# kuldeepbrd1/graspLDM

Measured on AMD Instinct MI355X. Metric: grasps/sec whole-node (1024-pt cloud, 100 DDIM steps), higher is better.
Workload: dtype f32 (GEMMs as split-f16 x3 partial products on the f16 matrix pipe, f32 accumulation; GroupNorm / LayerNorm / attention / scheduler in f32); 1 GPU; LDM mode, 256 synthetic 1024-pt clouds per GPU x 20 grasps, 100 DDIM steps: BASELINE.json configs[2] per GPU (configs[3] = this per-GPU workload on 8 GPUs); experiment=fpc, clouds_per_gpu=256, grasps_per_cloud=20, points=1024, ddim_steps=100, encoder=PVCNNEncoder (shipped fpc config), parallelism=cloud-sharded x1, weights=synthetic recipe seed 0, streams=3

## Files before the change

### graspldm_amd/csrc/conv3d.hip

```cpp
#include "mfma_core.h"
#include "voxel_geom.h"

namespace {

#ifdef GLDM_DEBUG_KNOBS
__device__ long long g_c3_stamp[32];
#define GLDM_C3_STAMP(i) \
  do { if (blockIdx.x == 5 && blockIdx.y == (gridDim.y >> 1) && threadIdx.x == 0) g_c3_stamp[i] = (long long)__builtin_readcyclecounter(); } while (0)
#else
#define GLDM_C3_STAMP(i) do {} while (0)
#endif

template <int CTRL>
__device__ __forceinline__ float c3_dpp_mov(float x) {
  return __int_as_float(__builtin_amdgcn_update_dpp(0, __float_as_int(x), CTRL, 0xf, 0xf, false));
}
__device__ __forceinline__ float row16_sum(float x) {
  x += c3_dpp_mov<0xB1>(x);
  x += c3_dpp_mov<0x4E>(x);
  x += c3_dpp_mov<0x141>(x);
  x += c3_dpp_mov<0x140>(x);
  return x;
}

constexpr int kConvThreads = 256;

__host__ __device__ constexpr bool brick_vec4(int r) { return r <= 24; }
__host__ __device__ constexpr int brick_zp(int r) { return brick_vec4(r) ? r + 8 : r + 2; }
__host__ __device__ constexpr int brick_row_stride(int r) {
  return ((6 * 6 * brick_zp(r) + 31) / 32 * 32 + 16) - 32 >= 6 * 6 * brick_zp(r) ? (6 * 6 * brick_zp(r) + 31) / 32 * 32 - 16
                                                                                 : (6 * 6 * brick_zp(r) + 31) / 32 * 32 + 16;
}

template <int MT, int NTW, int JN>
__global__ __launch_bounds__(kConvThreads, 2) void conv3d_k3_kernel(const float *__restrict__ x,
                                                                    const float *__restrict__ wp,
                                                                    const float *__restrict__ bias, int cin, int cout,
                                                                    int r_arg, float *__restrict__ y,
                                                                    float *__restrict__ partial, int cout_total, int co0,
                                                                    int out_cl) {
  constexpr int r = 4 * NTW;
  (void)r_arg;
  extern __shared__ float lds[];
  __builtin_amdgcn_s_setprio(3);
  GLDM_C3_STAMP(0);
  const int tid = threadIdx.x, wave = tid >> 6, lane = tid & 63;
  const int col = lane & 15, kq = lane >> 4;
  const int bpr = r / kBrick;
  const int bx0 = (blockIdx.x / bpr) * kBrick, by0 = (blockIdx.x % bpr) * kBrick;
  const int b = blockIdx.y;
  constexpr bool kVec = brick_vec4(r);
  constexpr int r3 = r * r * r, zp = brick_zp(r), bv = 36 * zp, bvp = brick_row_stride(r);
  const int cblocks = (cin + 15) >> 4, kblocks = 27 * cblocks;
  x += (size_t)b * cin * r3;
  y += out_cl ? (size_t)b * cout_total * r3 + co0 : ((size_t)b * cout_total + co0) * r3;
  const WStream wv(wp, lane);
  const lds_f *l3 = (const lds_f *)lds;

  int obase[NTW], gvox[NTW];
#pragma unroll
  for (int ni = 0; ni < NTW; ++ni) {
    const int o = 16 * (wave * NTW + ni) + col;
    const int iz = o % r, ixy = o / r, ix = ixy >> 2, iy = ixy & 3;
    obase[ni] = (ix * 6 + iy) * zp + iz + (kVec ? 3 : 0) + kq * bvp;
    gvox[ni] = ((bx0 + ix) * r + by0 + iy) * r + iz;
  }
  f32x4 acc[MT][NTW];
#pragma unroll
  for (int mi = 0; mi < MT; ++mi) {
    f32x4 bvv;
#pragma unroll
    for (int q = 0; q < 4; ++q) bvv[q] = bias[min(16 * mi + 4 * kq + q, cout - 1)];
#pragma unroll
    for (int ni = 0; ni < NTW; ++ni) acc[mi][ni] = bvv;
  }

  constexpr int kSlotsRow = r / 4, kSlots = 36 * kSlotsRow;
  static_assert(!kVec || kSlots <= kConvThreads, "one interior slot per thread");
  constexpr int SQ = kVec ? 1 : (36 * (4 * NTW + 2) + kConvThreads - 1) / kConvThreads;
  constexpr int kStageCh = JN == 1 ? 4 : 16;
  int s_lds[SQ], s_glb[SQ];
#pragma unroll
  for (int q = 0; q < SQ; ++q) {
    const int rem = tid + q * kConvThreads;
    s_lds[q] = -1;
    s_glb[q] = -1;
    if (kVec) {
      if (rem < kSlots) {
        const int ixy = rem / kSlotsRow, k = rem - ixy * kSlotsRow;
        const int gx = bx0 + ixy / 6 - 1, gy = by0 + ixy % 6 - 1;
        s_lds[q] = ixy * zp + 4 * (k + 1);
        if ((unsigned)gx < (unsigned)r && (unsigned)gy < (unsigned)r) s_glb[q] = (gx * r + gy) * r + 4 * k;
      }
    } else if (rem < bv) {
      s_lds[q] = rem;
      const int ixy = rem / zp, izp = rem - ixy * zp;
      const int gx = bx0 + ixy / 6 - 1, gy = by0 + ixy % 6 - 1, gz = izp - 1;
      if ((unsigned)gx < (unsigned)r && (unsigned)gy < (unsigned)r && (unsigned)gz < (unsigned)r)
        s_glb[q] = (gx * r + gy) * r + gz;
    }
  }
  if constexpr (kVec) {
    const f32x4 z4 = f32x4{0.f, 0.f, 0.f, 0.f};
    if (tid < 72) {
      float *lc = lds + (tid >> 1) * zp + ((tid & 1) ? 4 * (kSlotsRow + 1) : 0);
#pragma unroll
      for (int ci = 0; ci < kStageCh; ++ci) *reinterpret_cast<f32x4 *>(lc + ci * bvp) = z4;
    }
    if (s_lds[0] >= 0 && s_glb[0] < 0) {
      float *lc = lds + s_lds[0];
#pragma unroll
      for (int ci = 0; ci < kStageCh; ++ci) *reinterpret_cast<f32x4 *>(lc + ci * bvp) = z4;
    }
  }
  float stg[kVec ? 1 : SQ][kVec ? 1 : kStageCh];
  f32x4 stv[kVec ? kStageCh : 1];
  const __amdgpu_buffer_rsrc_t xrs = __builtin_amdgcn_make_buffer_rsrc(const_cast<float *>(x), 0, cin * r3 * 4, 0x00020000);
  auto stage_load = [&](int cb) {
    if constexpr (kVec) {
      const int g0 = s_glb[0] >= 0 ? s_glb[0] : 0;
#pragma unroll
      for (int ci = 0; ci < kStageCh; ++ci)
        stv[ci] = __builtin_bit_cast(f32x4, __builtin_amdgcn_raw_buffer_load_b128(xrs, ((cb * 16 + ci) * r3 + g0) * 4, 0, 0));
    } else {
      const float *xc = x + (size_t)(cb * 16) * r3;
#pragma unroll
      for (int q = 0; q < SQ; ++q)
#pragma unroll
        for (int ci = 0; ci < kStageCh; ++ci) {
          stg[q][ci] = 0.f;
          if (s_glb[q] >= 0 && cb * 16 + ci < cin) stg[q][ci] = xc[(size_t)ci * r3 + s_glb[q]];
        }
    }
  };
  auto stage_store = [&]() {
    if constexpr (kVec) {
      if (s_glb[0] >= 0) {
        float *lc = lds + s_lds[0];
#pragma unroll
        for (int ci = 0; ci < kStageCh; ++ci) *reinterpret_cast<f32x4 *>(lc + ci * bvp) = stv[ci];
      }
    } else {
#pragma unroll
      for (int q = 0; q < SQ; ++q)
        if (s_lds[q] >= 0) {
          float *lc = lds + s_lds[q];
#pragma unroll
          for (int ci = 0; ci < kStageCh; ++ci) lc[ci * bvp] = stg[q][ci];
        }
    }
  };
  constexpr int kStageLoads = SQ * kStageCh;
  constexpr bool kLate = r <= 12 && kStageLoads <= 32;
  constexpr bool kPipe = SQ <= 4;
  GLDM_C3_STAMP(1);
  if (kPipe) stage_load(0);
  GLDM_C3_STAMP(2);
  for (int cb = 0; cb < cblocks; ++cb) {
    __syncthreads();
    if (cb < 3) GLDM_C3_STAMP(3 + 4 * cb);
    if (!kPipe) stage_load(cb);
    stage_store();
    if (cb < 3) GLDM_C3_STAMP(4 + 4 * cb);
    if (kPipe && !kLate && cb + 1 < cblocks) stage_load(cb + 1);
    __builtin_amdgcn_sched_barrier(0);
    __syncthreads();
    if (cb < 3) GLDM_C3_STAMP(5 + 4 * cb);
    f32x4 a_cur[MT], a_nxt[MT];
#pragma unroll
    for (int mi = 0; mi < MT; ++mi) a_cur[mi] = wv[((size_t)mi * kblocks + cb) * 64];
    float bf[NTW], bn[NTW];
#pragma unroll
    for (int ni = 0; ni < NTW; ++ni) bf[ni] = l3[obase[ni]];
    __builtin_amdgcn_s_setprio(0);
    for (int tap = 0; tap < 27; ++tap) {
#ifdef GLDM_DEBUG_KNOBS
      if (cb < 2 && (tap == 1 || tap == 2 || tap == 14)) GLDM_C3_STAMP(14 + 3 * cb + (tap == 1 ? 0 : (tap == 2 ? 1 : 2)));
#endif
      if (kLate && tap == 25 && cb + 1 < cblocks) stage_load(cb + 1);
      const int tn = tap + 1 < 27 ? tap + 1 : tap;
#pragma unroll
      for (int mi = 0; mi < MT; ++mi) a_nxt[mi] = wv[((size_t)mi * kblocks + tn * cblocks + cb) * 64];
      __builtin_amdgcn_sched_barrier(0);
      const int toff = ((tap / 9) * 6 + (tap / 3) % 3) * zp + tap % 3;
      const int tnoff = ((tn / 9) * 6 + (tn / 3) % 3) * zp + tn % 3;
#pragma unroll
      for (int j = 0; j < JN; ++j) {
        const int noff = j + 1 < JN ? toff + 4 * (j + 1) * bvp : tnoff;
#pragma unroll
        for (int ni = 0; ni < NTW; ++ni) bn[ni] = l3[obase[ni] + noff];
#pragma unroll
        for (int mi = 0; mi < MT; ++mi)
#pragma unroll
          for (int ni = 0; ni < NTW; ++ni)
            acc[mi][ni] = __builtin_amdgcn_mfma_f32_16x16x4f32(a_cur[mi][j], bf[ni], acc[mi][ni], 0, 0, 0);
#pragma unroll
        for (int ni = 0; ni < NTW; ++ni) bf[ni] = bn[ni];
      }
#pragma unroll
      for (int mi = 0; mi < MT; ++mi) a_cur[mi] = a_nxt[mi];
    }
    __builtin_amdgcn_s_setprio(3);
    if (cb < 3) GLDM_C3_STAMP(6 + 4 * cb);
  }
  __syncthreads();
  GLDM_C3_STAMP(20);
  float *s_part = lds;
#pragma unroll
  for (int mi = 0; mi < MT; ++mi) {
#pragma unroll
    for (int q = 0; q < 4; ++q) {
      const int co = 16 * mi + 4 * kq + q;
      float s = 0.f, s2 = 0.f;
#pragma unroll
      for (int ni = 0; ni < NTW; ++ni) {
        const float v = acc[mi][ni][q];
        s += v;
        s2 += v * v;
      }
      s = row16_sum(s);
      s2 = row16_sum(s2);
      if (col == 0 && co < cout) {
        s_part[(wave * MT * 16 + co) * 2] = s;
        s_part[(wave * MT * 16 + co) * 2 + 1] = s2;
      }
    }
  }
  GLDM_C3_STAMP(24);
  __syncthreads();
  GLDM_C3_STAMP(25);
  if (tid < cout) {
    float s = 0.f, s2 = 0.f;
    for (int w = 0; w < 4; ++w) {
      s += s_part[(w * MT * 16 + tid) * 2];
      s2 += s_part[(w * MT * 16 + tid) * 2 + 1];
    }
    float *p = partial + (((size_t)b * gridDim.x + blockIdx.x) * cout_total + co0 + tid) * 2;
    p[0] = s;
    p[1] = s2;
  }
  GLDM_C3_STAMP(26);
  if (out_cl) {
#pragma unroll
    for (int ni = 0; ni < NTW; ++ni)
#pragma unroll
      for (int mi = 0; mi < MT; ++mi)
        if (16 * mi + 4 * kq < cout) *reinterpret_cast<f32x4 *>(y + (size_t)gvox[ni] * cout_total + 16 * mi + 4 * kq) = acc[mi][ni];
  } else {
#pragma unroll
    for (int mi = 0; mi < MT; ++mi)
#pragma unroll
      for (int q = 0; q < 4; ++q) {
        const int co = 16 * mi + 4 * kq + q;
        if (co < cout) {
#pragma unroll
          for (int ni = 0; ni < NTW; ++ni) y[(size_t)co * r3 + gvox[ni]] = acc[mi][ni][q];
        }
      }
  }
  GLDM_C3_STAMP(21);
}


constexpr int kPairs = 14;

__device__ __forceinline__ float c3_wave_max(float x) {
#pragma unroll
  for (int off = 32; off >= 1; off >>= 1) x = fmaxf(x, __shfl_xor(x, off, 64));
  return x;
}

template <int MT, int R, int ZB, int WAVES, bool ACT = false>
__global__ __launch_bounds__(64 * WAVES, (ZB * 16 / WAVES / 16 >= 6) ? 1 : 2) void conv3d_k3_pl_kernel(const float *__restrict__ x,
                                                                                      const float *__restrict__ wp3,
                                                                                      const float *__restrict__ bias, int cin,
                                                                                      int cout, float *__restrict__ y,
                                                                                      float *__restrict__ partial,
                                                                                      const float *__restrict__ in_coef,
                                                                                      int out_cl) {
  constexpr int r = R, NTW = ZB / WAVES, kThreads = 64 * WAVES, kZParts = R / ZB;
  constexpr int GM = MT % 3 == 0 ? 3 : (MT % 4 == 0 ? 4 : (MT % 2 == 0 ? 2 : 1));
  constexpr int GN = NTW % 3 == 0 ? 3 : (NTW % 2 == 0 ? 2 : 1);
  static_assert(R % ZB == 0 && ZB % WAVES == 0, "whole n-tiles per wave");
  constexpr int MG = MT / GM, NG = NTW / GN;
  constexpr int zp = ZB + 2, nvox = 36 * zp, r3 = r * r * r;
  constexpr int hs = (nvox + 15) & ~15;
  constexpr int kItems = 2 * nvox, kRounds = (kItems + kThreads - 1) / kThreads;
  constexpr bool kDB = R == 24 && ZB == 24;
  constexpr bool kRanged = !ACT;
  extern __shared__ float lds[];
  GLDM_C3_STAMP(0);
  __builtin_amdgcn_s_setprio(3);
  const int tid = threadIdx.x, wave = tid >> 6, lane = tid & 63;
  const int col = lane & 15, kq = lane >> 4;
  const int bpr = r / kBrick;
  const int bxy = blockIdx.x / kZParts, bz0 = (blockIdx.x % kZParts) * ZB;
  const int bx0 = (bxy / bpr) * kBrick, by0 = (bxy % bpr) * kBrick;
  const int b = blockIdx.y;
  const int cblocks = (cin + 15) >> 4, kblocks = kPairs * cblocks;
  x += (size_t)b * cin * r3;
  y += (size_t)b * cout * r3;
  const WStream wv(wp3, lane);
  constexpr int kSet = kSplit * 2 * hs;
  lds_u4 *pl0 = (lds_u4 *)lds;

  int vb[NTW];
#pragma unroll
  for (int ni = 0; ni < NTW; ++ni) {
    const int o = 16 * (wave * NTW + ni) + col;
    const int iz = o % ZB, ixy = o / ZB, ix = ixy >> 2, iy = ixy & 3;
    vb[ni] = (ix * 6 + iy) * zp + iz + (kq & 1) * hs;
  }
  f32x4 acc[MT][NTW];
#pragma unroll
  for (int mi = 0; mi < MT; ++mi) {
    f32x4 bvv;
#pragma unroll
    for (int q = 0; q < 4; ++q) bvv[q] = bias[16 * mi + 4 * kq + q];
#pragma unroll
    for (int ni = 0; ni < NTW; ++ni) acc[mi][ni] = bvv;
  }
  int s_lds[kRounds], s_glb[kRounds];
#pragma unroll
  for (int q = 0; q < kRounds; ++q) {
    const int it = tid + q * kThreads;
    s_lds[q] = -1;
    s_glb[q] = -1;
    if (it < kItems) {
      const int h = it / nvox, v = it - h * nvox;
      const int ixy = v / zp, izp = v - ixy * zp;
      const int gx = bx0 + ixy / 6 - 1, gy = by0 + ixy % 6 - 1, gz = bz0 + izp - 1;
      s_lds[q] = h * hs + v;
      if ((unsigned)gx < (unsigned)r && (unsigned)gy < (unsigned)r && (unsigned)gz < (unsigned)r)
        s_glb[q] = (gx * r + gy) * r + gz + 8 * h * r3;
    }
  }
  {
    const u32x4 z4 = u32x4{0u, 0u, 0u, 0u};
#pragma unroll
    for (int q = 0; q < kRounds; ++q)
      if (s_lds[q] >= 0 && s_glb[q] < 0) {
#pragma unroll
        for (int k = 0; k < kSplit; ++k) {
          pl0[k * 2 * hs + s_lds[q]] = z4;
          if constexpr (kDB) pl0[kSet + k * 2 * hs + s_lds[q]] = z4;
        }
      }
  }
  float stg[kRounds][8];
  auto stage_load = [&](int cb) {
    const float *xc = x + (size_t)(cb * 16) * r3;
#pragma unroll
    for (int q = 0; q < kRounds; ++q) {
      const int g0 = s_glb[q] >= 0 ? s_glb[q] : 0;
#pragma unroll
      for (int j = 0; j < 8; ++j) stg[q][j] = xc[(size_t)j * r3 + g0];
    }
  };
  float *s_coef = lds + (kDB ? 2 : 1) * kSet * 4;
  if constexpr (ACT) {
    for (int i = tid; i < 2 * cin; i += kThreads) s_coef[i] = in_coef[(size_t)b * cin * 2 + i];
  }
  unsigned s_run_u = 0x3f800000u;
  float *rng = s_coef;
  auto stage_store = [&](int cb) {
    lds_u4 *pl = pl0 + (kDB ? (cb & 1) * kSet : 0);
#pragma unroll
    for (int q = 0; q < kRounds; ++q)
      if (s_glb[q] >= 0) {
        if constexpr (kRanged) {
          const float inv_run = __uint_as_float((254u << 23) - s_run_u);
#pragma unroll
          for (int j = 0; j < 8; ++j) stg[q][j] *= inv_run;
        }
        if constexpr (ACT) {
          const int h = (tid + q * kThreads) / nvox;
          const f32x4 *cf = reinterpret_cast<const f32x4 *>(s_coef + 2 * (16 * cb + 8 * h));
#pragma unroll
          for (int j2 = 0; j2 < 4; ++j2) {
            const f32x4 c4 = cf[j2];
            const float t0 = fmaf(stg[q][2 * j2], c4[0], c4[1]), t1 = fmaf(stg[q][2 * j2 + 1], c4[2], c4[3]);
            stg[q][2 * j2] = t0 * __builtin_amdgcn_rcpf(1.0f + __builtin_amdgcn_exp2f(-1.44269504088896340736f * t0));
            stg[q][2 * j2 + 1] = t1 * __builtin_amdgcn_rcpf(1.0f + __builtin_amdgcn_exp2f(-1.44269504088896340736f * t1));
          }
        }
        u32x4 planes[kSplit];
        split_planes8(stg[q], planes);
#pragma unroll
        for (int k = 0; k < kSplit; ++k) pl[k * 2 * hs + s_lds[q]] = planes[k];
      }
  };
  GLDM_C3_STAMP(1);
  stage_load(0);
  GLDM_C3_STAMP(2);
  for (int cb = 0; cb < cblocks; ++cb) {
    if constexpr (kRanged) {
      float mx = 0.f;
#pragma unroll
      for (int q = 0; q < kRounds; ++q)
        if (s_glb[q] >= 0) {
#pragma unroll
          for (int j = 0; j < 8; ++j) mx = fmaxf(mx, fabsf(stg[q][j]));
        }
      mx = c3_wave_max(mx);
      if (lane == 0) rng[wave] = mx;
    }
    if (!kDB || kRanged || cb == 0) __syncthreads();
    if constexpr (kRanged) {
      float mx = 0.f;
#pragma unroll
      for (int w8 = 0; w8 < WAVES; ++w8) mx = fmaxf(mx, rng[w8]);
      const unsigned need = __builtin_amdgcn_readfirstlane(__float_as_uint(range_pow2(mx)));
      const unsigned s_new = (cb == 0 || need > s_run_u) ? need : s_run_u;
      if (s_new != s_run_u) {
        const float f = __uint_as_float(s_run_u) * pow2_inv(__uint_as_float(s_new));
#pragma unroll
        for (int mi = 0; mi < MT; ++mi)
#pragma unroll
          for (int ni = 0; ni < NTW; ++ni) acc[mi][ni] *= f;
        s_run_u = s_new;
      }
    }
    if (cb < 3) GLDM_C3_STAMP(3 + 4 * cb);
    stage_store(cb);
    if (cb + 1 < cblocks) stage_load(cb + 1);
    __builtin_amdgcn_sched_barrier(0);
    if (cb < 3) GLDM_C3_STAMP(4 + 4 * cb);
    __syncthreads();
    if (cb < 3) GLDM_C3_STAMP(5 + 4 * cb);
    const lds_u4 *pl = pl0 + (kDB ? (cb & 1) * kSet : 0);
    u32x4 a[2][GM][kSplit];
    auto load_a = [&](int buf, int step) {
      const int p = step / MG, mg = step - p * MG;
#pragma unroll
      for (int mi = 0; mi < GM; ++mi)
#pragma unroll
        for (int k = 0; k < kSplit; ++k)
          a[buf][mi][k] = wv.raw_at((((GM * mg + mi) * kblocks + cb * kPairs + p) * kSplit) * 1024, k * 1024);
    };
    load_a(0, 0);
    __builtin_amdgcn_s_setprio(0);
    constexpr int kSteps = kPairs * MG;
    constexpr int kUnits = kPairs * NG;
    constexpr bool kBPre = NG > 1;
    u32x4 bs[kBPre ? 2 : 1][GN][kSplit];
    auto load_b = [&](int buf, int unit) {
      const int p = unit / NG, ng = unit - p * NG;
      const int ta = 2 * p, tb = 2 * p + 1 < 27 ? 2 * p + 1 : 26;
      const int offa = ((ta / 9) * 6 + (ta / 3) % 3) * zp + ta % 3, offb = ((tb / 9) * 6 + (tb / 3) % 3) * zp + tb % 3;
      const int toff = (kq >> 1) ? offb : offa;
#pragma unroll
      for (int q = 0; q < GN; ++q)
#pragma unroll
        for (int k = 0; k < kSplit; ++k) bs[buf][q][k] = pl[k * 2 * hs + vb[GN * ng + q] + toff];
    };
    if (kBPre) load_b(0, 0);
    for (int p0 = 0; p0 < kPairs; p0 += 2) {
#pragma unroll
      for (int pu = 0; pu < 2; ++pu) {
        const int p = p0 + pu;
#pragma unroll
        for (int ng = 0; ng < NG; ++ng) {
          const int unit = p * NG + ng;
          const int bcur = kBPre ? ((pu * NG + ng) & 1) : 0;
          if (kBPre) load_b(bcur ^ 1, unit + 1 < kUnits ? unit + 1 : unit);
          else load_b(0, unit);
#pragma unroll
          for (int mg = 0; mg < MG; ++mg) {
            const int step = p * MG + mg;
            const int cur = (pu * MG + mg) & 1;
            if (ng == 0) load_a(cur ^ 1, step + 1 < kSteps ? step + 1 : step);
            __builtin_amdgcn_sched_barrier(0);
#pragma unroll
            for (int mi = 0; mi < GM; ++mi)
#pragma unroll
              for (int q = 0; q < GN; ++q)
                acc[GM * mg + mi][GN * ng + q] = mfma_split(a[cur][mi], bs[bcur][q], acc[GM * mg + mi][GN * ng + q]);
            __builtin_amdgcn_sched_barrier(0);
          }
        }
      }
    }
    if (cb < 3) GLDM_C3_STAMP(6 + 4 * cb);
    __builtin_amdgcn_s_setprio(3);
  }
  __syncthreads();
  GLDM_C3_STAMP(20);
  if constexpr (kRanged) {
    if (s_run_u != 0x3f800000u) {
      const float s_run = __uint_as_float(s_run_u);
#pragma unroll
      for (int mi = 0; mi < MT; ++mi)
#pragma unroll
        for (int ni = 0; ni < NTW; ++ni) acc[mi][ni] *= s_run;
    }
  }
  float *s_part = lds;
#pragma unroll
  for (int mi = 0; mi < MT; ++mi) {
#pragma unroll
    for (int q = 0; q < 4; ++q) {
      const int co = 16 * mi + 4 * kq + q;
      float s = 0.f, s2 = 0.f;
#pragma unroll
      for (int ni = 0; ni < NTW; ++ni) {
        const float v = acc[mi][ni][q];
        s += v;
        s2 += v * v;
      }
      s = row16_sum(s);
      s2 = row16_sum(s2);
      if (col == 0) {
        s_part[(wave * MT * 16 + co) * 2] = s;
        s_part[(wave * MT * 16 + co) * 2 + 1] = s2;
      }
    }
  }
  __syncthreads();
  if (tid < cout) {
    float s = 0.f, s2 = 0.f;
    for (int w = 0; w < WAVES; ++w) {
      s += s_part[(w * MT * 16 + tid) * 2];
      s2 += s_part[(w * MT * 16 + tid) * 2 + 1];
    }
    float *p = partial + (((size_t)b * (gridDim.x / kZParts) + bxy) * cout + tid) * 2;
    if constexpr (kZParts == 1) {
      p[0] = s;
      p[1] = s2;
    } else {
      atomicAdd(p, s);
      atomicAdd(p + 1, s2);
    }
  }
  int gvox[NTW];
  {
    int lane_o = lane;
    asm volatile("" : "+v"(lane_o));
#pragma unroll
    for (int ni = 0; ni < NTW; ++ni) {
      const int o = 16 * (wave * NTW + ni) + (lane_o & 15);
      const int iz = o % ZB, ixy = o / ZB, ix = ixy >> 2, iy = ixy & 3;
      gvox[ni] = ((bx0 + ix) * r + by0 + iy) * r + bz0 + iz;
    }
  }
  if (out_cl) {
#pragma unroll
    for (int ni = 0; ni < NTW; ++ni)
#pragma unroll
      for (int mi = 0; mi < MT; ++mi)
        *reinterpret_cast<f32x4 *>(y + (size_t)gvox[ni] * cout + 16 * mi + 4 * kq) = acc[mi][ni];
  } else {
#pragma unroll
    for (int mi = 0; mi < MT; ++mi)
#pragma unroll
      for (int q = 0; q < 4; ++q) {
        const int co = 16 * mi + 4 * kq + q;
#pragma unroll
        for (int ni = 0; ni < NTW; ++ni) y[(size_t)co * r3 + gvox[ni]] = acc[mi][ni][q];
      }
  }
  GLDM_C3_STAMP(21);
}

template <int MT, int R, int CIN, int WAVES>
__global__ __launch_bounds__(64 * WAVES, 4) void conv3d_k3_fewch_sp_kernel(const float *__restrict__ x,
                                                                           const float *__restrict__ wp3,
                                                                           const float *__restrict__ bias,
                                                                           float *__restrict__ y,
                                                                           float *__restrict__ partial) {
  constexpr int r = R, NTW = R / WAVES, kThreads = 64 * WAVES, zp = R + 2, nvox = 36 * zp, r3 = r * r * r;
  static_assert(R % WAVES == 0, "whole n-tiles per wave");
  constexpr int K = 27 * CIN, KB = (K + 31) / 32, cout = 16 * MT;
  constexpr int cs = nvox + ((nvox & 31) == 0 ? 8 : 0);
  extern __shared__ float lds[];
  const int tid = threadIdx.x, wave = tid >> 6, lane = tid & 63;
  const int col = lane & 15, g = lane >> 4;
  const int bpr = r / kBrick;
  const int bx0 = (blockIdx.x / bpr) * kBrick, by0 = (blockIdx.x % bpr) * kBrick;
  const int b = blockIdx.y;
  x += (size_t)b * CIN * r3;
  y += (size_t)b * cout * r3;
  float mx = 0.f;
  for (int i = tid; i < CIN * nvox; i += kThreads) {
    const int ci = i / nvox, v = i - ci * nvox;
    const int ixy = v / zp, izp = v - ixy * zp;
    const int gx = bx0 + ixy / 6 - 1, gy = by0 + ixy % 6 - 1, gz = izp - 1;
    float val = 0.f;
    if ((unsigned)gx < (unsigned)r && (unsigned)gy < (unsigned)r && (unsigned)gz < (unsigned)r)
      val = x[(size_t)ci * r3 + (gx * r + gy) * r + gz];
    lds[ci * cs + v] = val;
    mx = fmaxf(mx, fabsf(val));
  }
  float *rng = lds + CIN * cs;
  mx = c3_wave_max(mx);
  if (lane == 0) rng[wave] = mx;
  int vb[NTW], gvox[NTW];
#pragma unroll
  for (int ni = 0; ni < NTW; ++ni) {
    const int o = 16 * (wave * NTW + ni) + col;
    const int iz = o % r, ixy = o / r, ix = ixy >> 2, iy = ixy & 3;
    vb[ni] = (ix * 6 + iy) * zp + iz;
    gvox[ni] = ((bx0 + ix) * r + by0 + iy) * r + iz;
  }
  const WStream wv(wp3, lane);
  const lds_f *l3 = (const lds_f *)lds;
  __syncthreads();
  float s_in;
  {
    float m8 = 0.f;
#pragma unroll
    for (int w8 = 0; w8 < WAVES; ++w8) m8 = fmaxf(m8, rng[w8]);
    s_in = range_pow2(__uint_as_float(__builtin_amdgcn_readfirstlane(__float_as_uint(m8))));
  }
  const float inv_in = pow2_inv(s_in);
  f32x4 acc[MT][NTW];
#pragma unroll
  for (int mi = 0; mi < MT; ++mi) {
    const f32x4 bvv = *reinterpret_cast<const f32x4 *>(bias + 16 * mi + 4 * g) * inv_in;
#pragma unroll
    for (int ni = 0; ni < NTW; ++ni) acc[mi][ni] = bvv;
  }
#pragma unroll
  for (int kb = 0; kb < KB; ++kb) {
    u32x4 a[MT][kSplit];
#pragma unroll
    for (int mi = 0; mi < MT; ++mi)
#pragma unroll
      for (int pl = 0; pl < kSplit; ++pl) a[mi][pl] = wv.raw_at(((mi * KB + kb) * kSplit) * 1024, pl * 1024);
    int off[8];
#pragma unroll
    for (int j = 0; j < 8; ++j) {
      const int k = 32 * kb + 8 * g + j;
      const int tap = k / CIN, ci = k - tap * CIN;
      off[j] = k < K ? ci * cs + ((tap / 9) * 6 + (tap / 3) % 3) * zp + tap % 3 : 0;
    }
    float v[2][8];
#pragma unroll
    for (int j = 0; j < 8; ++j) v[0][j] = l3[vb[0] + off[j]];
#pragma unroll
    for (int ni = 0; ni < NTW; ++ni) {
      if (ni + 1 < NTW) {
#pragma unroll
        for (int j = 0; j < 8; ++j) v[(ni + 1) & 1][j] = l3[vb[ni + 1] + off[j]];
      }
      u32x4 b3[kSplit];
#pragma unroll
      for (int j = 0; j < 8; ++j) v[ni & 1][j] *= inv_in;
      split_planes8(v[ni & 1], b3);
#pragma unroll
      for (int mi = 0; mi < MT; ++mi) acc[mi][ni] = mfma_split(a[mi], b3, acc[mi][ni]);
    }
  }
  if (s_in != 1.0f) {
#pragma unroll
    for (int mi = 0; mi < MT; ++mi)
#pragma unroll
      for (int ni = 0; ni < NTW; ++ni) acc[mi][ni] *= s_in;
  }
  __syncthreads();
  float *s_part = lds;
#pragma unroll
  for (int mi = 0; mi < MT; ++mi) {
#pragma unroll
    for (int q = 0; q < 4; ++q) {
      const int co = 16 * mi + 4 * g + q;
      float s = 0.f, s2 = 0.f;
#pragma unroll
      for (int ni = 0; ni < NTW; ++ni) {
        const float v = acc[mi][ni][q];
        s += v;
        s2 += v * v;
      }
      s = row16_sum(s);
      s2 = row16_sum(s2);
      if (col == 0) {
        s_part[(wave * MT * 16 + co) * 2] = s;
        s_part[(wave * MT * 16 + co) * 2 + 1] = s2;
      }
    }
  }
  __syncthreads();
  if (tid < cout) {
    float s = 0.f, s2 = 0.f;
    for (int w = 0; w < WAVES; ++w) {
      s += s_part[(w * MT * 16 + tid) * 2];
      s2 += s_part[(w * MT * 16 + tid) * 2 + 1];
    }
    float *p = partial + (((size_t)b * gridDim.x + blockIdx.x) * cout + tid) * 2;
    p[0] = s;
    p[1] = s2;
  }
#pragma unroll
  for (int mi = 0; mi < MT; ++mi)
#pragma unroll
    for (int q = 0; q < 4; ++q) {
      const int co = 16 * mi + 4 * g + q;
#pragma unroll
      for (int ni = 0; ni < NTW; ++ni) y[(size_t)co * r3 + gvox[ni]] = acc[mi][ni][q];
    }
}

template <int MT, int NTW, int JN>
int launch_conv_jn(const float *x, const float *wp, const float *bias, int b, int cin, int cout, int r, float *y,
                float *partial, hipStream_t s, int cout_total, int co0, int out_cl) {
  const size_t lds_bytes = (size_t)16 * brick_row_stride(r) * sizeof(float);
  struct Tag {};
  gldm_dev::allow_dynamic_lds<Tag>(reinterpret_cast<const void *>(&conv3d_k3_kernel<MT, NTW, JN>), (int)lds_bytes);
  const int bpr = r / kBrick;
  hipLaunchKernelGGL((conv3d_k3_kernel<MT, NTW, JN>), dim3(bpr * bpr, b), dim3(kConvThreads), lds_bytes, s, x, wp, bias,
                     cin, cout, r, y, partial, cout_total, co0, out_cl);
  return hipGetLastError() == hipSuccess ? GLDM_OK : GLDM_ERR_LAUNCH;
}

__global__ __launch_bounds__(256) void conv3d_k3_generic_kernel(const float *__restrict__ x, const float *__restrict__ w,
                                                                const float *__restrict__ bias, int cin, int cout, int r,
                                                                float *__restrict__ y, float *__restrict__ partial) {
  __shared__ float s_red[2][4];
  const int bpr = bricks_per_axis(r), r3 = r * r * r, nvox = 16 * r;
  const int bx0 = (blockIdx.x / bpr) * kBrick, by0 = (blockIdx.x % bpr) * kBrick, b = blockIdx.y;
  x += (size_t)b * cin * r3;
  y += (size_t)b * cout * r3;
  const int tid = threadIdx.x;
  for (int co = 0; co < cout; ++co) {
    float s = 0.f, s2 = 0.f;
    for (int v = tid; v < nvox; v += 256) {
      const int iz = v % r, ixy = v / r, gx = bx0 + (ixy >> 2), gy = by0 + (ixy & 3);
      if (gx >= r || gy >= r) continue;
      float acc = bias[co];
      for (int ci = 0; ci < cin; ++ci) {
        const float *xc = x + (size_t)ci * r3;
        const float *wc = w + ((size_t)co * cin + ci) * 27;
#pragma unroll
        for (int tap = 0; tap < 27; ++tap) {
          const int nx = gx + tap / 9 - 1, ny = gy + (tap / 3) % 3 - 1, nz = iz + tap % 3 - 1;
          if ((unsigned)nx < (unsigned)r && (unsigned)ny < (unsigned)r && (unsigned)nz < (unsigned)r)
            acc = fmaf(wc[tap], xc[(nx * r + ny) * r + nz], acc);
        }
      }
      y[(size_t)co * r3 + (gx * r + gy) * r + iz] = acc;
      s += acc;
      s2 += acc * acc;
    }
    for (int off = 32; off >= 1; off >>= 1) {
      s += __shfl_xor(s, off, 64);
      s2 += __shfl_xor(s2, off, 64);
    }
    __syncthreads();
    if ((tid & 63) == 0) { s_red[0][tid >> 6] = s; s_red[1][tid >> 6] = s2; }
    __syncthreads();
    if (tid == 0) {
      float *p = partial + (((size_t)b * gridDim.x + blockIdx.x) * cout + co) * 2;
      p[0] = s_red[0][0] + s_red[0][1] + s_red[0][2] + s_red[0][3];
      p[1] = s_red[1][0] + s_red[1][1] + s_red[1][2] + s_red[1][3];
    }
  }
}

}

GLDM_API long long gldm_conv3d_partial_floats(int b, int cout, int r) {
  if (b <= 0 || cout <= 0 || r <= 0) return -1;
  const long long bpr = bricks_per_axis(r);
  return (long long)b * bpr * bpr * cout * 2;
}

template <int MT, int NTW>
int launch_conv(const float *x, const float *wp, const float *bias, int b, int cin, int cout, int r, float *y,
                float *partial, hipStream_t s, int out_cl, int cout_total = -1, int co0 = 0) {
  if (cout_total < 0) cout_total = cout;
  return cin <= 4 ? launch_conv_jn<MT, NTW, 1>(x, wp, bias, b, cin, cout, r, y, partial, s, cout_total, co0, out_cl)
                  : launch_conv_jn<MT, NTW, 4>(x, wp, bias, b, cin, cout, r, y, partial, s, cout_total, co0, out_cl);
}

template <int MH, int NTW>
int launch_conv_halves(const float *x, const float *wp, const float *bias, int b, int cin, int cout, int r, float *y,
                       float *partial, hipStream_t s, int out_cl) {
  const size_t kblocks = 27 * (size_t)((cin + 15) >> 4);
  const int half = 16 * MH;
  const int rc = launch_conv<MH, NTW>(x, wp, bias, b, cin, half, r, y, partial, s, out_cl, cout, 0);
  if (rc != GLDM_OK) return rc;
  return launch_conv<MH, NTW>(x, wp + (size_t)MH * kblocks * 256, bias + half, b, cin, cout - half, r, y, partial, s, out_cl, cout, half);
}

#define GLDM_CONV_F32_LIST(X, H)                                                                                          \
  X(3, 6)                                                               \
  X(6, 3)                                                                                                \
  X(2, 8)                                                                                      \
  X(3, 8)                                                                                          \
  X(4, 4)                                                                                                \
  X(8, 2)                                                                                                \
         \
  X(2, 4)                                                                                                \
  X(4, 2)                                                                                                 \
  X(1, 4)                                                                                                \
  X(2, 2)                                                                                                 \
  X(4, 1)                                                                                                 \
  X(8, 1)                                                                                                \
   \
  H(4, 8, 2)                                                                                                               \
  H(16, 2, 8)                                                                                            \
  H(8, 4, 4)

static int conv_f32_plan(int cin, int cout, int r) {
  if (cin <= 0 || cout <= 0 || r <= 0) return GLDM_ERR_UNSUPPORTED;
  if (r % 4 || (size_t)16 * brick_row_stride(r) * 4 > 160 * 1024) return GLDM_ERR_UNSUPPORTED;
  const int mt = (cout + 15) / 16, ntw = r / 4;
#define GLDM_CONV_CASE(M, N) if (mt == M && ntw == N) return GLDM_OK;
#define GLDM_CONV_HALVES(M, N, MH) GLDM_CONV_CASE(M, N)
  GLDM_CONV_F32_LIST(GLDM_CONV_CASE, GLDM_CONV_HALVES)
#undef GLDM_CONV_CASE
#undef GLDM_CONV_HALVES
  return GLDM_ERR_UNSUPPORTED;
}

static int conv3d_k3_impl(const float *x, const float *w_packed, const float *bias, int b, int cin, int cout, int r,
                          float *y, float *partial, int out_cl, gldm_stream_t stream) {
  if (!x || !w_packed || !bias || !y || !partial || b <= 0 || cin <= 0 || cout <= 0 || r <= 0)
    return GLDM_ERR_INVALID_ARG;
  if (out_cl && cout % 4) return GLDM_ERR_UNSUPPORTED;
  if (conv_f32_plan(cin, cout, r) != GLDM_OK) return GLDM_ERR_UNSUPPORTED;
  hipStream_t s = reinterpret_cast<hipStream_t>(stream);
  const int mt = (cout + 15) / 16, ntw = r / 4;
#ifdef GLDM_DEBUG_KNOBS
  struct StampDump {
    hipStream_t s; int cin, cout, r;
    ~StampDump() {
      if (!getenv("GLDM_C3_STAMP")) return;
      long long h[32];
      (void)hipStreamSynchronize(s);
      (void)hipMemcpyFromSymbol(h, HIP_SYMBOL(g_c3_stamp), sizeof(h));
      printf("conv3d %d->%d @%d: setup %lld, stage0 issue %lld", cin, cout, r, h[1] - h[0], h[2] - h[1]);
      for (int cb = 0; cb < (cin + 15) / 16 && cb < 3; ++cb)
        printf(" | cb%d: wait %lld store %lld barrier %lld taps %lld", cb, h[3 + 4 * cb] - (cb ? h[2 + 4 * cb] : h[2]),
               h[4 + 4 * cb] - h[3 + 4 * cb], h[5 + 4 * cb] - h[4 + 4 * cb], h[6 + 4 * cb] - h[5 + 4 * cb]);
      printf(" | epilogue %lld (stats %lld, barrier %lld, partials %lld, stores %lld), total %lld", h[21] - h[20], h[24] - h[20],
             h[25] - h[24], h[26] - h[25], h[21] - h[26], h[21] - h[0]);
      for (int cb = 0; cb < 2; ++cb)
        printf(" | cb%d taps: first %lld, second %lld, 2..13 %lld", cb, h[14 + 3 * cb] - h[5 + 4 * cb],
               h[15 + 3 * cb] - h[14 + 3 * cb], h[16 + 3 * cb] - h[15 + 3 * cb]);
      printf("\n");
    }
  } dump{s, cin, cout, r};
#endif
#define GLDM_CONV_CASE(M, N) \
  if (mt == M && ntw == N) return launch_conv<M, N>(x, w_packed, bias, b, cin, cout, r, y, partial, s, out_cl);
#define GLDM_CONV_HALVES(M, N, MH) \
  if (mt == M && ntw == N) return launch_conv_halves<MH, N>(x, w_packed, bias, b, cin, cout, r, y, partial, s, out_cl);
  GLDM_CONV_F32_LIST(GLDM_CONV_CASE, GLDM_CONV_HALVES)
#undef GLDM_CONV_CASE
#undef GLDM_CONV_HALVES
  return GLDM_ERR_UNSUPPORTED;
}

GLDM_API int gldm_conv3d_k3(const float *x, const float *w_packed, const float *bias, int b, int cin, int cout, int r,
                            float *y, float *partial, gldm_stream_t stream) {
  return conv3d_k3_impl(x, w_packed, bias, b, cin, cout, r, y, partial, 0, stream);
}

GLDM_API int gldm_conv3d_k3_cl(const float *x, const float *w_packed, const float *bias, int b, int cin, int cout, int r,
                               float *y_cl, float *partial, gldm_stream_t stream) {
  return conv3d_k3_impl(x, w_packed, bias, b, cin, cout, r, y_cl, partial, 1, stream);
}

template <int MT, int R, int ZB, int WAVES, bool ACT>
int launch_conv_pl_act(const float *x, const float *wp3, const float *bias, int b, int cin, int cout, float *y, float *partial,
                       const float *in_coef, int out_cl, hipStream_t s) {
  const size_t lds_bytes = (size_t)(R == 24 && ZB == 24 ? 2 : 1) * kSplit * 2 * ((36 * (ZB + 2) + 15) & ~15) * 16 +
                           (ACT ? (size_t)2 * cin * sizeof(float) : 64 );
  struct Tag {};
  gldm_dev::allow_dynamic_lds<Tag>(reinterpret_cast<const void *>(&conv3d_k3_pl_kernel<MT, R, ZB, WAVES, ACT>), (int)lds_bytes);
  const int bpr = R / kBrick;
  if (R != ZB) {
    if (hipMemsetAsync(partial, 0, (size_t)b * bpr * bpr * cout * 2 * sizeof(float), s) != hipSuccess) return GLDM_ERR_LAUNCH;
  }
  hipLaunchKernelGGL((conv3d_k3_pl_kernel<MT, R, ZB, WAVES, ACT>), dim3(bpr * bpr * (R / ZB), b), dim3(64 * WAVES), lds_bytes,
                     s, x, wp3, bias, cin, cout, y, partial, in_coef, out_cl);
  return hipGetLastError() == hipSuccess ? GLDM_OK : GLDM_ERR_LAUNCH;
}
template <int MT, int R, int ZB, int WAVES>
int launch_conv_pl(const float *x, const float *wp3, const float *bias, int b, int cin, int cout, float *y, float *partial,
                   const float *in_coef, int out_cl, hipStream_t s) {
  return in_coef ? launch_conv_pl_act<MT, R, ZB, WAVES, true>(x, wp3, bias, b, cin, cout, y, partial, in_coef, out_cl, s)
                 : launch_conv_pl_act<MT, R, ZB, WAVES, false>(x, wp3, bias, b, cin, cout, y, partial, nullptr, out_cl, s);
}

#define GLDM_CONV_SPLIT_LIST(X)                                                                 \
  X(48, 24, 3, 24, 24, 8)                                                                        \
  X(96, 12, 6, 12, 12, 4)                                                                        \
                            \
  X(32, 32, 2, 32, 32, 8)                                                                        \
  X(64, 32, 4, 32, 32, 8)                                                                        \
  X(32, 16, 2, 16, 16, 4)                                                                        \
  X(64, 16, 4, 16, 16, 4)                                                                        \
  X(128, 16, 8, 16, 16, 8)                                                                       \
  X(64, 8, 4, 8, 8, 4)                                                                           \
  X(128, 8, 8, 8, 8, 4)                                                                          \
  X(256, 8, 16, 8, 8, 8)                                                                         \
  X(128, 4, 8, 4, 4, 4)

constexpr bool conv_split_fewch(int cin, int cout, int r) { return cin == 3 && cout == 48 && r == 24; }

static int conv_split_plan(int cin, int cout, int r) {
  if (cin <= 0 || cout <= 0 || r <= 0) return GLDM_ERR_UNSUPPORTED;
  if (conv_split_fewch(cin, cout, r)) return GLDM_OK;
  if (cin % 16) return GLDM_ERR_UNSUPPORTED;
#define GLDM_CONV_CASE(C, RR, MT, R, ZB, WAVES) if (cout == C && r == RR) return GLDM_OK;
  GLDM_CONV_SPLIT_LIST(GLDM_CONV_CASE)
#undef GLDM_CONV_CASE
  return GLDM_ERR_UNSUPPORTED;
}

static int conv3d_k3_f16x2_impl(const float *x, const float *in_coef, const float *w_split, const float *bias, int b, int cin,
                                 int cout, int r, float *y, float *partial, int out_cl, gldm_stream_t stream) {
  if (!x || !w_split || !bias || !y || !partial || b <= 0 || cin <= 0 || cout <= 0 || r <= 0) return GLDM_ERR_INVALID_ARG;
  if ((in_coef || out_cl) && cin % 16) return GLDM_ERR_UNSUPPORTED;
  if (conv_split_plan(cin, cout, r) != GLDM_OK) return GLDM_ERR_UNSUPPORTED;
  hipStream_t s = reinterpret_cast<hipStream_t>(stream);
  if (conv_split_fewch(cin, cout, r)) {
    constexpr int kZp = 26, kNvox = 36 * kZp;
    const size_t lds_bytes = (size_t)3 * (kNvox + ((kNvox & 31) == 0 ? 8 : 0)) * sizeof(float) + 64;
    hipLaunchKernelGGL((conv3d_k3_fewch_sp_kernel<3, 24, 3, 8>), dim3(36, b), dim3(512), lds_bytes, s, x, w_split, bias, y, partial);
    return hipGetLastError() == hipSuccess ? GLDM_OK : GLDM_ERR_LAUNCH;
  }
#ifdef GLDM_DEBUG_KNOBS
  struct StampDump {
    hipStream_t s; int cin, cout, r, b;
    ~StampDump() {
      if (!getenv("GLDM_C3_STAMP")) return;
      long long h[32];
      (void)hipStreamSynchronize(s);
      (void)hipMemcpyFromSymbol(h, HIP_SYMBOL(g_c3_stamp), sizeof(h));
      printf("conv3d split %d->%d @%d b=%d: setup %lld, stage0 issue %lld", cin, cout, r, b, h[1] - h[0], h[2] - h[1]);
      for (int cb = 0; cb < cin / 16 && cb < 3; ++cb)
        printf(" | cb%d: wait %lld store %lld barrier %lld taps %lld", cb, h[3 + 4 * cb] - (cb ? h[2 + 4 * cb] : h[2]),
               h[4 + 4 * cb] - h[3 + 4 * cb], h[5 + 4 * cb] - h[4 + 4 * cb], h[6 + 4 * cb] - h[5 + 4 * cb]);
      printf(" | epilogue %lld, total %lld\n", h[21] - h[20], h[21] - h[0]);
    }
  } dump{s, cin, cout, r, b};
#endif
#define GLDM_CONV_CASE(C, RR, MT, R, ZB, WAVES) \
  if (cout == C && r == RR) return launch_conv_pl<MT, R, ZB, WAVES>(x, w_split, bias, b, cin, cout, y, partial, in_coef, out_cl, s);
  GLDM_CONV_SPLIT_LIST(GLDM_CONV_CASE)
#undef GLDM_CONV_CASE
  return GLDM_ERR_UNSUPPORTED;
}

GLDM_API int gldm_conv3d_k3_supported(int kind, int cin, int cout, int r) {
  if (kind == GLDM_CONV3D_F32) return conv_f32_plan(cin, cout, r);
  if (kind == GLDM_CONV3D_F16X2) return conv_split_plan(cin, cout, r);
  return GLDM_ERR_INVALID_ARG;
}

GLDM_API int gldm_conv3d_k3_f16x2(const float *x, const float *w_split, const float *bias, int b, int cin, int cout, int r,
                                   float *y, float *partial, gldm_stream_t stream) {
  return conv3d_k3_f16x2_impl(x, nullptr, w_split, bias, b, cin, cout, r, y, partial, 0, stream);
}

GLDM_API int gldm_conv3d_k3_f16x2_gn(const float *x, const float *in_coef, const float *w_split, const float *bias, int b,
                                      int cin, int cout, int r, float *y, float *partial, int out_channel_last,
                                      gldm_stream_t stream) {
  return conv3d_k3_f16x2_impl(x, in_coef, w_split, bias, b, cin, cout, r, y, partial, out_channel_last ? 1 : 0, stream);
}

GLDM_API int gldm_conv3d_k3_generic(const float *x, const float *w, const float *bias, int b, int cin, int cout, int r,
                                    float *y, float *partial, gldm_stream_t stream) {
  if (!x || !w || !bias || !y || !partial || b <= 0 || cin <= 0 || cout <= 0 || r <= 0) return GLDM_ERR_INVALID_ARG;
  hipLaunchKernelGGL(conv3d_k3_generic_kernel, dim3(bricks_per_cloud(r), b), dim3(256), 0, reinterpret_cast<hipStream_t>(stream), x, w,
                     bias, cin, cout, r, y, partial);
  return hipGetLastError() == hipSuccess ? GLDM_OK : GLDM_ERR_LAUNCH;
}
```

### graspldm_amd/csrc/voxel_geom.h

```cpp
#pragma once
#include <hip/hip_runtime.h>

namespace {

constexpr int kBrick = 4;
constexpr int bricks_per_axis(int r) { return (r + kBrick - 1) / kBrick; }
constexpr int bricks_per_cloud(int r) { return bricks_per_axis(r) * bricks_per_axis(r); }

constexpr int kSumParts = 8;

__device__ __forceinline__ void trilinear_corners(float x, float y, float z, int r, float (&w)[8], int (&idx)[8]) {
  const int r2 = r * r;
  const float xl = floorf(x), yl = floorf(y), zl = floorf(z);
  const float xd1 = x - xl, yd1 = y - yl, zd1 = z - zl;
  const float xd0 = 1.0f - xd1, yd0 = 1.0f - yd1, zd0 = 1.0f - zd1;
  w[0] = xd0 * yd0 * zd0; w[1] = xd0 * yd0 * zd1; w[2] = xd0 * yd1 * zd0; w[3] = xd0 * yd1 * zd1;
  w[4] = xd1 * yd0 * zd0; w[5] = xd1 * yd0 * zd1; w[6] = xd1 * yd1 * zd0; w[7] = xd1 * yd1 * zd1;
  const int zh = zd1 > 0 ? 1 : 0, yh = yd1 > 0 ? r : 0, xh = xd1 > 0 ? r2 : 0;
  idx[0] = (int)xl * r2 + (int)yl * r + (int)zl;
  idx[1] = idx[0] + zh; idx[2] = idx[0] + yh; idx[3] = idx[2] + zh;
  idx[4] = idx[0] + xh; idx[5] = idx[4] + zh; idx[6] = idx[4] + yh; idx[7] = idx[6] + zh;
}

}
```

### graspldm_amd/voxel.py

```python
import torch

from . import _lib as L
from .r1d_pack import mfma_a_fragments

_F32, _F16X2 = 0, 1
CONV_ROW_TILE = 16
FIRST_VOXEL_CONV = (3, 48, 24)


def _instantiated(kind, cin, cout, r):
    return L.lib().gldm_conv3d_k3_supported(kind, int(cin), int(cout), int(r)) == 0


def conv_supported(cout, r):
    return cout % CONV_ROW_TILE == 0 and _instantiated(_F32, 1, cout, r)


def pack_conv3d(weight):
    cout, cin = weight.shape[:2]
    cpad = (cin + 15) // 16 * 16
    w = torch.zeros(cout, 27, cpad, dtype=torch.float32)
    w[:, :, :cin] = weight.detach().float().cpu().reshape(cout, cin, 27).permute(0, 2, 1)
    return mfma_a_fragments(w.reshape(cout, 27 * cpad))


def split_conv_supported(cin, cout, r):
    from .numerics import split_enabled
    if not _instantiated(_F16X2, cin, cout, r):
        return False
    if (cin, cout, r) == FIRST_VOXEL_CONV:
        return split_enabled()
    return split_enabled() or not conv_supported(cout, r)


def pack_conv3d_fewch_f16x2(weight):
    from .r1d_pack import mfma_a_fragments_f16x2
    cout, cin = weight.shape[:2]
    k = 27 * cin
    w = torch.zeros(cout, (k + 31) // 32 * 32, dtype=torch.float32)
    w[:, :k] = weight.detach().float().cpu().reshape(cout, cin, 27).permute(0, 2, 1).reshape(cout, k)
    return mfma_a_fragments_f16x2(w)


def pack_conv3d_f16x2(weight):
    from .r1d_pack import mfma_a_fragments_f16x2
    cout, cin = weight.shape[:2]
    cb = cin // 16
    w = torch.zeros(cout, cb, 14, 2, 16, dtype=torch.float32)
    wt = weight.detach().float().cpu().reshape(cout, cb, 16, 27)
    taps = torch.zeros(cout, cb, 16, 28)
    taps[..., :27] = wt
    w[:] = taps.reshape(cout, cb, 16, 14, 2).permute(0, 1, 3, 4, 2)
    return mfma_a_fragments_f16x2(w.reshape(cout, cb * 14 * 32))


class VoxelBranchPlan:

    def __init__(self, convs, device, r=None):
        from .r1d_pack import SplitRangeError
        self.split = [r is not None and split_conv_supported(c.in_channels, c.out_channels, r) for c in convs]
        self.generic = [r is not None and not conv_supported(c.out_channels, r) for c in convs]
        self.w = []
        for i, c in enumerate(convs):
            if self.split[i]:
                try:
                    self.w.append((pack_conv3d_fewch_f16x2(c.weight) if c.in_channels < 16 else pack_conv3d_f16x2(c.weight)).to(device))
                    continue
                except SplitRangeError:
                    self.split[i] = False
            self.w.append((c.weight.detach().float().contiguous() if self.generic[i] else pack_conv3d(c.weight)).to(device))


def _launch_conv(plan, i, conv, x, coef, b, r, cl, st):
    cin, cout = conv.in_channels, conv.out_channels
    y = torch.empty((b, cout, r, r, r), dtype=torch.float32, device=x.device)
    nf = L.lib().gldm_conv3d_partial_floats(b, cout, r)
    partial = torch.empty(int(nf), dtype=torch.float32, device=x.device)
    staged = plan.split[i] and cin % 16 == 0
    if staged and (coef is not None or cl):
        L.call("gldm_conv3d_k3_f16x2_gn", L.ptr(x), L.ptr(coef), L.ptr(plan.w[i]), L.ptr(conv.bias), b, cin, cout, r,
               L.ptr(y), L.ptr(partial), 1 if cl else 0, st)
    elif cl:
        assert coef is None
        L.call("gldm_conv3d_k3_cl", L.ptr(x), L.ptr(plan.w[i]), L.ptr(conv.bias), b, cin, cout, r, L.ptr(y), L.ptr(partial), st)
    else:
        assert coef is None
        entry = "gldm_conv3d_k3_generic" if plan.generic[i] else ("gldm_conv3d_k3_f16x2" if plan.split[i] else "gldm_conv3d_k3")
        L.call(entry, L.ptr(x), L.ptr(plan.w[i]), L.ptr(conv.bias), b, cin, cout, r, L.ptr(y), L.ptr(partial), st)
    return y, partial


def _next_conv_stages_norm(plan, convs, i, r):
    return plan.split[i + 1] and convs[i + 1].in_channels % 16 == 0 and r >= 16


def _groupnorm_coef(partial, gn, b, c, r, st):
    coef = torch.empty((b, c, 2), dtype=torch.float32, device=partial.device)
    L.call("gldm_groupnorm_coef", L.ptr(partial), L.ptr(gn.weight), L.ptr(gn.bias), b, c, r, gn.num_groups, float(gn.eps),
           L.ptr(coef), st)
    return coef


def run(plan, convs, norms, se, vox, norm_coords, point_feat, r):
    dev = vox.device
    b = vox.shape[0]
    st = L.current_stream(dev)
    x = vox.contiguous()
    coef = None
    chan_sum = None
    x_cl = False
    with torch.cuda.device(dev):
        for i, (conv, gn) in enumerate(zip(convs, norms)):
            cin, cout = conv.in_channels, conv.out_channels
            last = i == len(convs) - 1
            staged = plan.split[i] and cin % 16 == 0
            mfma32 = not plan.split[i] and not plan.generic[i]
            cl = last and (staged or mfma32) and cout % 4 == 0 and cout <= 256 and cout // gn.num_groups <= 64
            y, partial = _launch_conv(plan, i, conv, x, coef, b, r, cl, st)
            x_cl = cl
            foldable = (last or _next_conv_stages_norm(plan, convs, i, r)) and cout // gn.num_groups <= 64
            if foldable:
                coef = _groupnorm_coef(partial, gn, b, cout, r, st)
            else:
                coef = None
                if last and se is not None:
                    chan_sum = torch.empty((b, cout), dtype=torch.float32, device=dev)
                L.call("gldm_groupnorm_swish", L.ptr(y), L.ptr(partial), L.ptr(gn.weight), L.ptr(gn.bias), b, cout, r,
                       gn.num_groups, float(gn.eps), L.ptr(chan_sum) if (last and se is not None) else None, st)
            x = y
        c = x.shape[1]
        gate = None
        if se is not None:
            gate = torch.empty((b, c), dtype=torch.float32, device=dev)
            w1, w2 = se.fc[0].weight, se.fc[2].weight
            if x_cl:
                parts = int(L.lib().gldm_squeeze_parts())
                chan_sum = torch.empty((b, parts, c), dtype=torch.float32, device=dev)
                L.call("gldm_gn_swish_chan_sum_cl", L.ptr(x), L.ptr(coef), b, c, r, L.ptr(chan_sum), st)
                L.call("gldm_se_gate_parts", L.ptr(chan_sum), parts, L.ptr(w1), L.ptr(w2), b, c, w1.shape[0], r,
                       1 if se.use_relu else 0, L.ptr(gate), st)
            else:
                if coef is not None:
                    chan_sum = torch.empty((b, c), dtype=torch.float32, device=dev)
                    L.call("gldm_gn_swish_chan_sum", L.ptr(x), L.ptr(coef), b, c, r, L.ptr(chan_sum), st)
                L.call("gldm_se_gate", L.ptr(chan_sum), L.ptr(w1), L.ptr(w2), b, c, w1.shape[0], r,
                       1 if se.use_relu else 0, L.ptr(gate), st)
        n = norm_coords.shape[2]
        out = torch.empty((b, c, n), dtype=torch.float32, device=dev)
        pf = point_feat.contiguous() if point_feat is not None else None
        if x_cl:
            L.call("gldm_devoxelize_gn_cl_fused", L.ptr(norm_coords), L.ptr(x), L.ptr(coef), L.ptr(gate), L.ptr(pf), b, c, n, r,
                   L.ptr(out), st)
        elif coef is not None:
            L.call("gldm_devoxelize_gn_fused", L.ptr(norm_coords), L.ptr(x), L.ptr(coef), L.ptr(gate), L.ptr(pf), b, c, n, r,
                   L.ptr(out), st)
        else:
            L.call("gldm_devoxelize_fused", L.ptr(norm_coords), L.ptr(x), L.ptr(gate), L.ptr(pf), b, c, n, r, L.ptr(out), st)
    return out


def run_attention(plan, convs, norms, attn, se, vox, norm_coords, point_feat, r):
    from . import attention as A
    dev = vox.device
    b = vox.shape[0]
    st = L.current_stream(dev)
    x = vox.contiguous()
    coef = None
    with torch.cuda.device(dev):
        for i, (conv, gn) in enumerate(zip(convs, norms)):
            cout, last = conv.out_channels, i == len(convs) - 1
            y, partial = _launch_conv(plan, i, conv, x, coef, b, r, False, st)
            if last or (_next_conv_stages_norm(plan, convs, i, r) and cout // gn.num_groups <= 64):
                coef = _groupnorm_coef(partial, gn, b, cout, r, st)
            else:
                coef = None
                L.call("gldm_groupnorm_swish", L.ptr(y), L.ptr(partial), L.ptr(gn.weight), L.ptr(gn.bias), b, cout, r,
                       gn.num_groups, float(gn.eps), None, st)
            x = y
        c = x.shape[1]
        xa = torch.empty((b, c, r ** 3), dtype=torch.float32, device=dev)
        L.call("gldm_groupnorm_affine", L.ptr(x), L.ptr(coef), b, c, r, L.ptr(xa), st)
        pq, po = attn._packed(dev)
        h = A.run_conv(A.attention_core(A.run_conv(xa, pq), xa, xa), po)
        gate = None
        if se is not None:
            feat, chan_sum = A.groupnorm_swish_sum(h, attn.norm, add=xa)
            gate = torch.empty((b, c), dtype=torch.float32, device=dev)
            w1, w2 = se.fc[0].weight, se.fc[2].weight
            L.call("gldm_se_gate", L.ptr(chan_sum), L.ptr(w1), L.ptr(w2), b, c, w1.shape[0], r, 1 if se.use_relu else 0,
                   L.ptr(gate), st)
        else:
            feat = A.groupnorm_swish(h, attn.norm, add=xa)
        n = norm_coords.shape[2]
        out = torch.empty((b, c, n), dtype=torch.float32, device=dev)
        pf = point_feat.contiguous() if point_feat is not None else None
        L.call("gldm_devoxelize_fused", L.ptr(norm_coords), L.ptr(feat), L.ptr(gate), L.ptr(pf), b, c, n, r, L.ptr(out), st)
    return out
```

Baseline: 311,300 grasps/s.

## Remap conv3d workgroups so each XCD handles whole clouds; nontemporal output stores

Flattens the conv3d launch grid into one dimension and uses a brick_work mapping. Under that mapping, consecutive workgroup IDs, which round-robin across the 8 XCDs, land on different clouds, so each XCD keeps all bricks of a given cloud and its halo and weight data stay in that XCD's L2. Output stores in the pipelined kernel become nontemporal to avoid polluting cache. The GroupNorm staging threshold also drops from r>=16 to r>=12, so more layers fuse normalization into the next conv. The risks are that the remap assumes the hardware dispatches workgroups round-robin across XCDs, and that nontemporal stores could hurt when the next kernel reads the output soon after.

```diff
diff --git a/graspldm_amd/csrc/conv3d.hip b/graspldm_amd/csrc/conv3d.hip
--- a/graspldm_amd/csrc/conv3d.hip
+++ b/graspldm_amd/csrc/conv3d.hip
@@ -5,9 +5,11 @@
 
 #ifdef GLDM_DEBUG_KNOBS
 __device__ long long g_c3_stamp[32];
+#define GLDM_C3_STAMP_WG(brick, cloud, clouds) const bool c3_stamp_wg = (brick) == 5 && (cloud) == ((clouds) >> 1)
 #define GLDM_C3_STAMP(i) \
-  do { if (blockIdx.x == 5 && blockIdx.y == (gridDim.y >> 1) && threadIdx.x == 0) g_c3_stamp[i] = (long long)__builtin_readcyclecounter(); } while (0)
+  do { if (c3_stamp_wg && threadIdx.x == 0) g_c3_stamp[i] = (long long)__builtin_readcyclecounter(); } while (0)
 #else
+#define GLDM_C3_STAMP_WG(brick, cloud, clouds) do {} while (0)
 #define GLDM_C3_STAMP(i) do {} while (0)
 #endif
 
@@ -43,6 +45,7 @@
   (void)r_arg;
   extern __shared__ float lds[];
   __builtin_amdgcn_s_setprio(3);
+  GLDM_C3_STAMP_WG(blockIdx.x, blockIdx.y, gridDim.y);
   GLDM_C3_STAMP(0);
   const int tid = threadIdx.x, wave = tid >> 6, lane = tid & 63;
   const int col = lane & 15, kq = lane >> 4;
@@ -262,6 +265,9 @@
 }
 
 
+template <typename T>
+__device__ __forceinline__ void c3_store(T *p, T v) { __builtin_nontemporal_store(v, p); }
+
 constexpr int kPairs = 14;
 
 __device__ __forceinline__ float c3_wave_max(float x) {
@@ -277,7 +283,7 @@
                                                                                       int cout, float *__restrict__ y,
                                                                                       float *__restrict__ partial,
                                                                                       const float *__restrict__ in_coef,
-                                                                                      int out_cl) {
+                                                                                      int out_cl, int clouds) {
   constexpr int r = R, NTW = ZB / WAVES, kThreads = 64 * WAVES, kZParts = R / ZB;
   constexpr int GM = MT % 3 == 0 ? 3 : (MT % 4 == 0 ? 4 : (MT % 2 == 0 ? 2 : 1));
   constexpr int GN = NTW % 3 == 0 ? 3 : (NTW % 2 == 0 ? 2 : 1);
@@ -289,14 +295,16 @@
   constexpr bool kDB = R == 24 && ZB == 24;
   constexpr bool kRanged = !ACT;
   extern __shared__ float lds[];
+  constexpr int bpr = r / kBrick;
+  int b, unit;
+  brick_work(blockIdx.x, clouds, bpr * bpr * kZParts, b, unit);
+  GLDM_C3_STAMP_WG(unit, b, clouds);
   GLDM_C3_STAMP(0);
   __builtin_amdgcn_s_setprio(3);
   const int tid = threadIdx.x, wave = tid >> 6, lane = tid & 63;
   const int col = lane & 15, kq = lane >> 4;
-  const int bpr = r / kBrick;
-  const int bxy = blockIdx.x / kZParts, bz0 = (blockIdx.x % kZParts) * ZB;
+  const int bxy = unit / kZParts, bz0 = (unit % kZParts) * ZB;
   const int bx0 = (bxy / bpr) * kBrick, by0 = (bxy % bpr) * kBrick;
-  const int b = blockIdx.y;
   const int cblocks = (cin + 15) >> 4, kblocks = kPairs * cblocks;
   x += (size_t)b * cin * r3;
   y += (size_t)b * cout * r3;
@@ -523,7 +531,7 @@
       s += s_part[(w * MT * 16 + tid) * 2];
       s2 += s_part[(w * MT * 16 + tid) * 2 + 1];
     }
-    float *p = partial + (((size_t)b * (gridDim.x / kZParts) + bxy) * cout + tid) * 2;
+    float *p = partial + (((size_t)b * (bpr * bpr) + bxy) * cout + tid) * 2;
     if constexpr (kZParts == 1) {
       p[0] = s;
       p[1] = s2;
@@ -548,7 +556,7 @@
     for (int ni = 0; ni < NTW; ++ni)
 #pragma unroll
       for (int mi = 0; mi < MT; ++mi)
-        *reinterpret_cast<f32x4 *>(y + (size_t)gvox[ni] * cout + 16 * mi + 4 * kq) = acc[mi][ni];
+        c3_store(reinterpret_cast<f32x4 *>(y + (size_t)gvox[ni] * cout + 16 * mi + 4 * kq), acc[mi][ni]);
   } else {
 #pragma unroll
     for (int mi = 0; mi < MT; ++mi)
@@ -556,7 +564,7 @@
       for (int q = 0; q < 4; ++q) {
         const int co = 16 * mi + 4 * kq + q;
 #pragma unroll
-        for (int ni = 0; ni < NTW; ++ni) y[(size_t)co * r3 + gvox[ni]] = acc[mi][ni][q];
+        for (int ni = 0; ni < NTW; ++ni) c3_store(y + (size_t)co * r3 + gvox[ni], acc[mi][ni][q]);
       }
   }
   GLDM_C3_STAMP(21);
@@ -567,7 +575,7 @@
                                                                            const float *__restrict__ wp3,
                                                                            const float *__restrict__ bias,
                                                                            float *__restrict__ y,
-                                                                           float *__restrict__ partial) {
+                                                                           float *__restrict__ partial, int clouds) {
   constexpr int r = R, NTW = R / WAVES, kThreads = 64 * WAVES, zp = R + 2, nvox = 36 * zp, r3 = r * r * r;
   static_assert(R % WAVES == 0, "whole n-tiles per wave");
   constexpr int K = 27 * CIN, KB = (K + 31) / 32, cout = 16 * MT;
@@ -575,9 +583,10 @@
   extern __shared__ float lds[];
   const int tid = threadIdx.x, wave = tid >> 6, lane = tid & 63;
   const int col = lane & 15, g = lane >> 4;
-  const int bpr = r / kBrick;
-  const int bx0 = (blockIdx.x / bpr) * kBrick, by0 = (blockIdx.x % bpr) * kBrick;
-  const int b = blockIdx.y;
+  constexpr int bpr = r / kBrick;
+  int b, bxy;
+  brick_work(blockIdx.x, clouds, bpr * bpr, b, bxy);
+  const int bx0 = (bxy / bpr) * kBrick, by0 = (bxy % bpr) * kBrick;
   x += (size_t)b * CIN * r3;
   y += (size_t)b * cout * r3;
   float mx = 0.f;
@@ -686,7 +695,7 @@
       s += s_part[(w * MT * 16 + tid) * 2];
       s2 += s_part[(w * MT * 16 + tid) * 2 + 1];
     }
-    float *p = partial + (((size_t)b * gridDim.x + blockIdx.x) * cout + tid) * 2;
+    float *p = partial + (((size_t)b * (bpr * bpr) + bxy) * cout + tid) * 2;
     p[0] = s;
     p[1] = s2;
   }
@@ -873,8 +882,8 @@
   if (R != ZB) {
     if (hipMemsetAsync(partial, 0, (size_t)b * bpr * bpr * cout * 2 * sizeof(float), s) != hipSuccess) return GLDM_ERR_LAUNCH;
   }
-  hipLaunchKernelGGL((conv3d_k3_pl_kernel<MT, R, ZB, WAVES, ACT>), dim3(bpr * bpr * (R / ZB), b), dim3(64 * WAVES), lds_bytes,
-                     s, x, wp3, bias, cin, cout, y, partial, in_coef, out_cl);
+  hipLaunchKernelGGL((conv3d_k3_pl_kernel<MT, R, ZB, WAVES, ACT>), dim3(bpr * bpr * (R / ZB) * b), dim3(64 * WAVES), lds_bytes,
+                     s, x, wp3, bias, cin, cout, y, partial, in_coef, out_cl, b);
   return hipGetLastError() == hipSuccess ? GLDM_OK : GLDM_ERR_LAUNCH;
 }
 template <int MT, int R, int ZB, int WAVES>
@@ -919,7 +928,7 @@
   if (conv_split_fewch(cin, cout, r)) {
     constexpr int kZp = 26, kNvox = 36 * kZp;
     const size_t lds_bytes = (size_t)3 * (kNvox + ((kNvox & 31) == 0 ? 8 : 0)) * sizeof(float) + 64;
-    hipLaunchKernelGGL((conv3d_k3_fewch_sp_kernel<3, 24, 3, 8>), dim3(36, b), dim3(512), lds_bytes, s, x, w_split, bias, y, partial);
+    hipLaunchKernelGGL((conv3d_k3_fewch_sp_kernel<3, 24, 3, 8>), dim3(36 * b), dim3(512), lds_bytes, s, x, w_split, bias, y, partial, b);
     return hipGetLastError() == hipSuccess ? GLDM_OK : GLDM_ERR_LAUNCH;
   }
 #ifdef GLDM_DEBUG_KNOBS
diff --git a/graspldm_amd/csrc/voxel_geom.h b/graspldm_amd/csrc/voxel_geom.h
--- a/graspldm_amd/csrc/voxel_geom.h
+++ b/graspldm_amd/csrc/voxel_geom.h
@@ -6,6 +6,19 @@
 constexpr int kBrick = 4;
 constexpr int bricks_per_axis(int r) { return (r + kBrick - 1) / kBrick; }
 constexpr int bricks_per_cloud(int r) { return bricks_per_axis(r) * bricks_per_axis(r); }
+
+constexpr int kXcdLabels = 8;
+__host__ __device__ __forceinline__ void brick_work(int id, int clouds, int nb, int &cloud, int &brick) {
+  const int whole = clouds / kXcdLabels * kXcdLabels;
+  if (id < whole * nb) {
+    const int k = id / kXcdLabels;
+    cloud = id % kXcdLabels + kXcdLabels * (k / nb);
+    brick = k % nb;
+  } else {
+    cloud = id / nb;
+    brick = id % nb;
+  }
+}
 
 constexpr int kSumParts = 8;
 
diff --git a/graspldm_amd/voxel.py b/graspldm_amd/voxel.py
--- a/graspldm_amd/voxel.py
+++ b/graspldm_amd/voxel.py
@@ -91,7 +91,7 @@
 
 
 def _next_conv_stages_norm(plan, convs, i, r):
-    return plan.split[i + 1] and convs[i + 1].in_channels % 16 == 0 and r >= 16
+    return plan.split[i + 1] and convs[i + 1].in_channels % 16 == 0 and r >= 12
 
 
 def _groupnorm_coef(partial, gn, b, c, r, st):
```

After: 312,400 grasps/s, median of 6. About the same (+0.3%).
